# jwfoley/UniPeak

Measured on AMD Instinct MI355X. Metric: genome Gbp/s for KDE smoothing + region scan on hg19, at 1/2/4/8 MI355X, higher is better.
Workload: dtype f64

## Files before the change

include/unipeak_hip.h:

```cpp
#ifndef UNIPEAK_HIP_H
#define UNIPEAK_HIP_H

#include <stddef.h>
#include <stdint.h>

#ifdef __cplusplus
extern "C" {
#endif

#define UP_OK 0
#define UP_E_ARG (-1)
#define UP_E_HIP (-2)
#define UP_E_NOMEM (-3)
#define UP_E_STATE (-4)
#define UP_E_UNSUPPORTED (-5)
#define UP_E_NODEV (-6)
#define UP_E_INTERNAL (-7)

typedef struct up_ctx up_ctx;

typedef struct {
    uint16_t bw;
    uint16_t n_samples;
    int32_t nondir;
// ... 63 lines not shown
#define UP_MAX_IN_FLIGHT 5
int up_run_async(up_ctx *ctx);
int up_run_wait(up_ctx *ctx, uint64_t *n_regions);
int up_set_timing(up_ctx *ctx, int level);
int up_get_regions(up_ctx *ctx, up_region *out, uint32_t *counts, size_t cap);
int up_regions_view(up_ctx *ctx, const up_region **regions, const uint32_t **counts,
                    uint64_t *n);

int up_set_record_target(up_ctx *ctx, void *buf, uint64_t cap);
int up_host_register(up_ctx *ctx, void *ptr, uint64_t bytes);

int up_shift_scan(up_ctx *ctx, const uint64_t *region_idx, size_t n,
                  uint16_t max_shift, double *out);
int up_shift_best(up_ctx *ctx, const uint64_t *region_idx, size_t n,
                  uint16_t max_shift, uint16_t *best_shift, double *best_corr);

#define UP_INDEX_AUTO 0
#define UP_INDEX_NEVER 1
#define UP_INDEX_ALWAYS 2
int up_set_index_policy(up_ctx *ctx, int policy);
int up_invalidate_index(up_ctx *ctx);
int up_index_state(up_ctx *ctx, int *on, uint64_t *builds);
int up_last_stats_kind(up_ctx *ctx);
int up_scan_density(up_ctx *ctx, uint32_t *bytes_per_1024);
int up_hbm_copy_gbps(up_ctx *ctx, uint64_t bytes, int reps, double *gbps);
int up_timings(up_ctx *ctx, double *ms, int n);
int up_unit_profile(up_ctx *ctx, uint32_t unit, double *out_f, double *out_r,
                    uint32_t len);
#define UP_FLUSH_EVENT 0xFFFFFFFFu
int up_set_profile_capture(up_ctx *ctx, int on);
int up_unit_replay_profile(up_ctx *ctx, uint32_t unit, uint32_t *resync, uint64_t *n,
                           uint32_t *event, uint32_t *pos, double *score, uint64_t cap);
int up_unit_profile_range(up_ctx *ctx, uint32_t unit, uint64_t first, uint32_t count,
                          double *out_f, double *out_r);

#define UP_TIR_HOST 0xFFFFFFFFu
typedef struct up_tir up_tir;
int up_tir_open(int hip_device, up_tir **out);
void up_tir_close(up_tir *h);
int up_tir_set_stream(up_tir *h, uint32_t stream, uint64_t n, const uint64_t *key,
                      const uint32_t *count, const uint8_t *forward);
int up_tir_query(up_tir *h, uint32_t n_streams, uint64_t n_regions, const uint32_t *contig,
                 const uint32_t *left, const uint32_t *right, const uint8_t *forward,
                 uint32_t *first, uint32_t *end, uint32_t *hits);
int up_tir_timings(up_tir *h, double *ms, int n);

// ... 14 lines not shown
```

unipeak_amd/capi.py:

```python
import ctypes
import os

import numpy as np

_HERE = os.path.dirname(os.path.abspath(__file__))
LIB_PATH = os.environ.get("UNIPEAK_LIB") or os.path.join(_HERE, "lib", "libunipeak_hip.so")

UP_OK = 0
MAX_IN_FLIGHT = 5


class UpError(RuntimeError):
    def __init__(self, code, msg):
        super().__init__(f"{msg} (code {code})")
        self.code = code


class Params(ctypes.Structure):
    _fields_ = [
        ("bw", ctypes.c_uint16),
        ("n_samples", ctypes.c_uint16),
        ("nondir", ctypes.c_int32),
        ("background", ctypes.c_double),
        ("region_thr", ctypes.c_double),
# ... 19 lines not shown
        ("close_pos", ctypes.c_uint32),
        ("peak_score", ctypes.c_double),
        ("kurtosis", ctypes.c_double),
        ("corr", ctypes.c_double),
    ]


REGION_DTYPE = np.dtype([
    ("unit", "<u4"), ("left", "<u4"), ("right", "<u4"), ("peak", "<u4"),
    ("sum", "<u4"), ("nonctl_sum", "<u4"), ("accepted", "<i4"), ("close_pos", "<u4"),
    ("peak_score", "<f8"), ("kurtosis", "<f8"), ("corr", "<f8")])
assert REGION_DTYPE.itemsize == ctypes.sizeof(Region)

_lib = None

EXPORTS = [
    "up_version", "up_track_bits", "up_strerror", "up_device_count", "up_kernel_weights", "up_open",
    "up_close", "up_set_params", "up_add_unit", "up_unit_count", "up_unit_pack",
    "up_unit_scatter", "up_unit_synth", "up_unit_synth_offset", "up_unit_synth_ex", "up_unit_tag_total", "up_unit_set_last_add", "up_unit_last_add",
    "up_reset_units", "up_run", "up_get_regions", "up_regions_view", "up_shift_scan", "up_shift_best",
    "up_timings", "up_scan_density", "up_unit_profile", "up_hbm_copy_gbps", "up_set_record_target",
    "up_host_register", "up_unit_profile_range", "up_run_async", "up_run_wait", "up_set_timing",
    "up_set_profile_capture", "up_unit_replay_profile",
    "up_set_index_policy", "up_invalidate_index", "up_index_state", "up_last_stats_kind",
    "up_tir_open", "up_tir_close", "up_tir_set_stream", "up_tir_query", "up_tir_timings",
    "up_cm_open", "up_cm_close", "up_cm_add", "up_cm_collect", "up_cm_timings",
]
TIR_HOST = 0xFFFFFFFF
INDEX_AUTO, INDEX_NEVER, INDEX_ALWAYS = 0, 1, 2


def load_library(path=LIB_PATH):
    global _lib
    if _lib is not None:
        return _lib
    if not os.path.exists(path):
        raise OSError(f"{path} not built: run `python __graft_entry__.py` / tools/build.py")
    L = ctypes.CDLL(path)
    c = ctypes
    vp, u32p = c.c_void_p, c.POINTER(c.c_uint32)
    sig = {
        "up_version": (c.c_int, []),
        "up_track_bits": (c.c_int, []),
        "up_strerror": (c.c_char_p, [c.c_int]),
        "up_device_count": (c.c_int, [c.POINTER(c.c_int)]),
        "up_kernel_weights": (c.c_int, [c.c_uint16, c.c_double, vp]),
        "up_open": (c.c_int, [c.c_int, c.POINTER(vp)]),
# ... 9 lines not shown
                                           c.c_uint32, c.c_int32, c.c_int32, c.c_int32, c.c_int32]),
        "up_unit_synth_ex": (c.c_int, [vp, c.c_uint32, c.c_int32, c.c_uint16, c.c_uint64,
                                       c.c_uint32, c.c_int32, c.c_int32, c.c_int32, c.c_int32,
                                       c.c_uint64]),
        "up_unit_tag_total": (c.c_int, [vp, c.c_uint32, c.c_int32, c.c_uint16,
                                        c.POINTER(c.c_uint64)]),
        "up_unit_set_last_add": (c.c_int, [vp, c.c_uint32, c.c_uint32]),
        "up_unit_last_add": (c.c_int, [vp, c.c_uint32, u32p]),
        "up_reset_units": (c.c_int, [vp]),
        "up_run": (c.c_int, [vp, c.POINTER(c.c_uint64)]),
        "up_run_async": (c.c_int, [vp]),
        "up_run_wait": (c.c_int, [vp, c.POINTER(c.c_uint64)]),
        "up_set_timing": (c.c_int, [vp, c.c_int]),
        "up_get_regions": (c.c_int, [vp, vp, vp, c.c_size_t]),
        "up_regions_view": (c.c_int, [vp, c.POINTER(vp), c.POINTER(vp), c.POINTER(c.c_uint64)]),
        "up_shift_scan": (c.c_int, [vp, vp, c.c_size_t, c.c_uint16, vp]),
        "up_shift_best": (c.c_int, [vp, vp, c.c_size_t, c.c_uint16, vp, vp]),
        "up_timings": (c.c_int, [vp, vp, c.c_int]),
        "up_scan_density": (c.c_int, [vp, u32p]),
        "up_set_index_policy": (c.c_int, [vp, c.c_int]),
        "up_invalidate_index": (c.c_int, [vp]),
        "up_index_state": (c.c_int, [vp, c.POINTER(c.c_int), c.POINTER(c.c_uint64)]),
        "up_last_stats_kind": (c.c_int, [vp]),
        "up_unit_profile": (c.c_int, [vp, c.c_uint32, vp, vp, c.c_uint32]),
        "up_hbm_copy_gbps": (c.c_int, [vp, c.c_uint64, c.c_int, c.POINTER(c.c_double)]),
        "up_set_record_target": (c.c_int, [vp, vp, c.c_uint64]),
        "up_host_register": (c.c_int, [vp, vp, c.c_uint64]),
        "up_unit_profile_range": (c.c_int, [vp, c.c_uint32, c.c_uint64, c.c_uint32, vp, vp]),
        "up_set_profile_capture": (c.c_int, [vp, c.c_int]),
        "up_unit_replay_profile": (c.c_int, [vp, c.c_uint32, u32p, c.POINTER(c.c_uint64), vp, vp, vp,
                                             c.c_uint64]),
        "up_tir_open": (c.c_int, [c.c_int, c.POINTER(vp)]),
        "up_tir_close": (None, [vp]),
        "up_tir_set_stream": (c.c_int, [vp, c.c_uint32, c.c_uint64, vp, vp, vp]),
        "up_tir_query": (c.c_int, [vp, c.c_uint32, c.c_uint64, vp, vp, vp, vp, vp, vp, vp]),
        "up_tir_timings": (c.c_int, [vp, vp, c.c_int]),
        "up_cm_open": (c.c_int, [c.c_int, c.c_uint32, vp, c.POINTER(vp)]),
        "up_cm_close": (None, [vp]),
        "up_cm_add": (c.c_int, [vp, c.c_uint64, vp, vp, vp, vp]),
        "up_cm_collect": (c.c_int, [vp, c.c_int, c.POINTER(c.c_uint64), vp, vp, vp, vp, c.c_uint64]),
        "up_cm_timings": (c.c_int, [vp, vp, c.c_int]),
    }
    for name, (res, args) in sig.items():
        fn = getattr(L, name)
        fn.restype = res
        fn.argtypes = args
# ... 163 lines not shown

    def host_register(self, ptr, nbytes):
        _ck(self.L.up_host_register(self.ctx, ctypes.c_void_p(ptr), nbytes))

    def hbm_copy_gbps(self, nbytes=1 << 30, reps=5):
        v = ctypes.c_double()
        _ck(self.L.up_hbm_copy_gbps(self.ctx, nbytes, reps, ctypes.byref(v)))
        return v.value

    def set_index_policy(self, policy):
        _ck(self.L.up_set_index_policy(self.ctx, int(policy)))

    def invalidate_index(self):
        _ck(self.L.up_invalidate_index(self.ctx))

    def index_state(self):
        on, b = ctypes.c_int(0), ctypes.c_uint64(0)
        _ck(self.L.up_index_state(self.ctx, ctypes.byref(on), ctypes.byref(b)))
        return bool(on.value), int(b.value)

    def last_k3_kind(self):
        return int(self.L.up_last_stats_kind(self.ctx))

    def scan_density(self):
        v = ctypes.c_uint32()
        _ck(self.L.up_scan_density(self.ctx, ctypes.byref(v)))
        return v.value

    def timings(self):
        t = np.zeros(5, np.float64)
        _ck(self.L.up_timings(self.ctx, t.ctypes.data, 5))
        return t

    def profile(self, unit, length):
        f = np.zeros(length, np.float64)
        r = np.zeros(length, np.float64)
        _ck(self.L.up_unit_profile(self.ctx, unit, f.ctypes.data, r.ctypes.data, length))
        return f, r

    def profile_range(self, unit, first, count):
        f = np.zeros(count, np.float64)
        r = np.zeros(count, np.float64)
        _ck(self.L.up_unit_profile_range(self.ctx, unit, first, count, f.ctypes.data, r.ctypes.data))
        return f, r

    def profile_kernel_ms(self):
# ... 101 lines not shown
```

unipeak_amd/csrc/api.hip:

```cpp
#include <hip/hip_runtime.h>

#include <algorithm>
#include <unordered_map>
#include <chrono>
#include <cmath>
#include <condition_variable>
#include <deque>
#include <cstdio>
#include <cstring>
#include <map>
#include <mutex>
#include <thread>
#include <vector>

#include "../../include/unipeak_hip.h"
#include "kernels.h"

#include "kernels.hip"
#include "stats1.hip"
#include "emulate.hip"
#include "q11place.hip"
#include "wide.hip"

namespace upk {
const void *scan_kernel_nh1(int, bool, bool, int);
const void *scan_kernel_nh2(int, bool, bool, int);
const void *scan_kernel_nh3(int, bool, bool, int);
const void *scan_kernel_nh4(int, bool, bool, int);
const void *scan_kernel_nh5(int, bool, bool, int);
const void *scan_kernel_nh6(int, bool, bool, int);
const void *scan_kernel_nh7(int, bool, bool, int);
const void *scan_kernel_nh8(int, bool, bool, int);
const void *stats_kernel_nh1(int, bool, int);
const void *stats_kernel_nh2(int, bool, int);
const void *stats_kernel_nh3(int, bool, int);
const void *stats_kernel_nh4(int, bool, int);
const void *stats_kernel_nh5(int, bool, int);
const void *stats_kernel_nh6(int, bool, int);
const void *stats_kernel_nh7(int, bool, int);
const void *stats_kernel_nh8(int, bool, int);
const void *shift_kernel_nh1(int);
const void *shift_kernel_nh2(int);
const void *shift_kernel_nh3(int);
const void *shift_kernel_nh4(int);
const void *shift_kernel_nh5(int);
const void *shift_kernel_nh6(int);
const void *shift_kernel_nh7(int);
const void *shift_kernel_nh8(int);
static int window_nh(int bw) { return (bw + 64) / 64; }
static const void *scan_kernel_for(int bw, int pool, bool nd, bool prof, int mode) {
    switch (window_nh(bw)) {
    case 1: return scan_kernel_nh1(pool, nd, prof, mode);
    case 2: return scan_kernel_nh2(pool, nd, prof, mode);
    case 3: return scan_kernel_nh3(pool, nd, prof, mode);
    case 4: return scan_kernel_nh4(pool, nd, prof, mode);
    case 5: return scan_kernel_nh5(pool, nd, prof, mode);
    case 6: return scan_kernel_nh6(pool, nd, prof, mode);
    case 7: return scan_kernel_nh7(pool, nd, prof, mode);
    default: return scan_kernel_nh8(pool, nd, prof, mode);
    }
}
static const void *stats_kernel_for(int bw, int pool, bool nd, int one) {
    switch (window_nh(bw)) {
    case 1: return stats_kernel_nh1(pool, nd, one);
    case 2: return stats_kernel_nh2(pool, nd, one);
    case 3: return stats_kernel_nh3(pool, nd, one);
    case 4: return stats_kernel_nh4(pool, nd, one);
    case 5: return stats_kernel_nh5(pool, nd, one);
    case 6: return stats_kernel_nh6(pool, nd, one);
    case 7: return stats_kernel_nh7(pool, nd, one);
    default: return stats_kernel_nh8(pool, nd, one);
    }
// ... 76 lines not shown
        hipError_t e = hipHostMalloc((void **)&p, cap * sizeof(T), hipHostMallocMapped | hipHostMallocCoherent);
        if (e != hipSuccess) return e;
        e = hipHostGetDevicePointer((void **)&dev, p, 0);
        if (e == hipSuccess) n = cap;
        return e;
    }
    void release() {
        if (p) (void)hipHostFree(p);
        p = dev = nullptr;
        n = 0;
    }
};

constexpr int kSlots = UP_MAX_IN_FLIGHT;

}

struct up_ctx {
    int dev = 0;
    int ncu = 0;
    int k1a_per_cu = 3;
    int k1b_per_cu = 0;
    int k3_per_cu = 0;
    bool k3_one = true;
    bool use_graphs = true;
    hipStream_t k1a_stream = nullptr;
    hipStream_t chain[4] = {};
    int n_chain = 3;
    uint64_t nlaunch = 0;
    hipStream_t stream = nullptr;
    bool have_params = false;
    up_params p{};
    std::vector<uint8_t> ctl;
    std::vector<double> coef, kern;
    std::vector<int32_t> nc;
    DevBuf<double> d_kern, d_coef;
    DevBuf<int32_t> d_nc;
    DevBuf<uint8_t> d_ctl;
    DevBuf<uint32_t> d_wscreen;
    uint32_t wskip = 0;
    float fw[kScrHalo + 1] = {};
    float fthr = 0.f;
    bool q_ok = false;
    double q_alpha = 0.0, q_delta = 1.0;
    uint32_t qno = 0, qyes = 0;
    uint32_t ovf_max_all = 0;
// ... 39 lines not shown
        DevBuf<double> d_corr;
        void release() {
            d_info.release(); d_rec.release(); d_ovf_count.release(); d_ovf_rec.release(); d_head.release();
            d_cnt.release(); d_nreg.release(); d_bsum.release(); d_starts.release(); d_ends.release();
            d_runit.release(); d_peak_pos.release(); d_xlist.release(); d_xcount.release();
            d_xwcount.release(); d_xref.release(); d_peak_val.release(); d_spk.release(); d_corr.release();
        }
        uint8_t *target = nullptr;
        void *target_hostp = nullptr;
        uint64_t target_cap = 0;
        uint8_t *req_target = nullptr;
        void *req_target_hostp = nullptr;
        uint64_t req_target_cap = 0, req_last_nreg = 0;
        uint64_t req_reg_cap = 0;
        uint32_t req_ovf_cap = 0;
        int req_tl = 0;
        bool req_q11 = false;
        bool req_q11_place = false;
        bool lpending = false;
        int lrc = 0;
        uint64_t cap = 0;
        uint32_t ovf_cap = 0;
        int tl = 0;
        int k3_kind = -1;
        std::chrono::steady_clock::time_point t0;
        hipEvent_t ev[5] = {};
        hipEvent_t done = nullptr;
    } pass[kSlots];
    uint64_t seq_launched = 0, seq_done = 0;
    int cur_slot = 0;
    std::thread launcher;
    std::mutex lmu;
    std::condition_variable lcv;
    std::deque<int> lq;
    bool lbusy = false, lstop = false, use_launcher = true;
    hipEvent_t host_work = nullptr;
    DevBuf<uint32_t> d_resync, d_emu_n, d_emu_err, d_emu_counts, d_ring_hits, d_reg_hit, d_reg_hits;
    DevBuf<int32_t> d_unit_buffer;
    DevBuf<uint32_t> d_gunits, d_goff;
    DevBuf<uint32_t> d_gskip, d_gstop, d_emu_group;
    DevBuf<double> d_reg_f, d_reg_r;
    DevBuf<up_region> d_emu_out;
    DevBuf<double> d_ring_f, d_ring_r;
    bool prof_capture = false;
    uint64_t pf_cap = 1u << 20;
    DevBuf<uint32_t> d_pf_unit, d_pf_event, d_pf_pos;
// ... 29 lines not shown
    DevBuf<uint32_t> d_q11_stage_cnt;
    DevBuf<Q11Place> d_q11_tab;
    DevBuf<uint64_t> d_q11_scr;
    DevBuf<Q11Edit> d_q11_edit;
    DevBuf<uint32_t> d_q11_st, d_q11_en, d_q11_src;
    std::vector<std::pair<uint64_t, uint64_t>> q11_rep;
    std::vector<up_region> h_regions;
    std::vector<uint32_t> h_counts;
    std::vector<uint8_t> h_emulated;
    HostBuf<uint32_t> hp_head[kSlots];
    HostBuf<up_region> hp_regions[kSlots];
    HostBuf<uint32_t> hp_counts[kSlots];
    HostBuf<unsigned long long> hp_status[kSlots];
    void *target_hostp = nullptr;
    HostBuf<uint32_t> hp_scat[2];
    hipEvent_t scat_ev[2] = {};
    int scat_i = 0;
    uint64_t reg_cap = 1u << 16;
    uint8_t *target = nullptr;
    uint64_t target_cap = 0;
    void *target_host = nullptr;
    std::vector<void *> host_regs;
    uint64_t last_nreg = 0;
    int last_k3_kind = -1;
};

static bool busy(const up_ctx *c) { return c && c->seq_launched != c->seq_done; }

static void index_stale(up_ctx *c) { c->passes_on_tracks = 0; }

static void sync_all(up_ctx *c) {
    (void)hipStreamSynchronize(c->stream);
    (void)hipStreamSynchronize(c->k1a_stream);
    for (auto st : c->chain)
        if (st) (void)hipStreamSynchronize(st);
}

#define HIPCHK(x)                                                                   \
    do {                                                                            \
        hipError_t e_ = (x);                                                        \
        if (e_ != hipSuccess) {                                                     \
            fprintf(stderr, "unipeak_hip: %s failed: %s (%s:%d)\n", #x,             \
                    hipGetErrorString(e_), __FILE__, __LINE__);                     \
            return e_ == hipErrorOutOfMemory ? UP_E_NOMEM : UP_E_HIP;               \
        }                                                                           \
    } while (0)
// ... 20 lines not shown
int up_set_index_policy(up_ctx *c, int policy) {
    if (!c || policy < UP_INDEX_AUTO || policy > UP_INDEX_ALWAYS) return UP_E_ARG;
    if (busy(c)) return UP_E_STATE;
    c->index_policy = policy;
    return UP_OK;
}

int up_invalidate_index(up_ctx *c) {
    if (!c) return UP_E_ARG;
    if (busy(c)) return UP_E_STATE;
    for (Unit &u : c->units) u.cs_dirty = u.pool_dirty = true;
    index_stale(c);
    return UP_OK;
}

int up_index_state(up_ctx *c, int *on, uint64_t *builds) {
    if (!c) return UP_E_ARG;
    if (on) *on = c->index_on ? 1 : 0;
    if (builds) *builds = c->index_builds;
    return UP_OK;
}

int up_last_stats_kind(up_ctx *c) { return c ? c->last_k3_kind : -1; }

const char *up_strerror(int code) {
    switch (code) {
    case UP_OK: return "ok";
    case UP_E_ARG: return "bad argument";
    case UP_E_HIP: return "HIP runtime error";
    case UP_E_NOMEM: return "device memory exhausted";
    case UP_E_STATE: return "call out of order";
    case UP_E_UNSUPPORTED: return "configuration outside the GPU path";
    case UP_E_NODEV: return "no HIP device";
    case UP_E_INTERNAL: return "internal consistency check failed";
    default: return "unknown error";
    }
}

int up_device_count(int *n) {
    if (!n) return UP_E_ARG;
    int c = 0;
    if (hipGetDeviceCount(&c) != hipSuccess) c = 0;
    *n = c;
    return UP_OK;
}

// ... 5 lines not shown
        const double x2 = x * x;
        w[j] = 3 * (1 - x2) / 4;
        acc += w[j];
    }
    const double scale = sum / acc;
    for (int j = 0; j < 2 * (int)bw + 1; ++j) w[j] *= scale;
    return UP_OK;
}

int up_open(int hip_device, up_ctx **out) {
    if (!out) return UP_E_ARG;
    int n = 0;
    if (hipGetDeviceCount(&n) != hipSuccess || n == 0) return UP_E_NODEV;
    if (hip_device < 0 || hip_device >= n) return UP_E_ARG;
    up_ctx *c = new up_ctx();
    c->dev = hip_device;
    HIPCHK(hipSetDevice(hip_device));
    HIPCHK(hipDeviceGetAttribute(&c->ncu, hipDeviceAttributeMultiprocessorCount, hip_device));
    if (const char *e = getenv("UNIPEAK_K1A_PER_CU")) c->k1a_per_cu = atoi(e);
    if (const char *e = getenv("UNIPEAK_GRAPHS")) c->use_graphs = e[0] != '0';
    if (const char *e = getenv("UNIPEAK_K1B_PER_CU")) c->k1b_per_cu = atoi(e);
    if (const char *e = getenv("UNIPEAK_K3_PER_CU")) c->k3_per_cu = atoi(e);
    if (const char *e = getenv("UNIPEAK_K3_ONE")) c->k3_one = atoi(e) != 0;
    if (const char *e = getenv("UNIPEAK_CHAINS")) c->n_chain = std::min(4, std::max(1, atoi(e)));
    if (const char *e = getenv("UNIPEAK_LAUNCHER")) c->use_launcher = e[0] != '0';
    {
        int least = 0, greatest = 0;
        HIPCHK(hipDeviceGetStreamPriorityRange(&least, &greatest));
        const char *ep = getenv("UNIPEAK_CTX_PRIO");
        HIPCHK(hipStreamCreateWithPriority(&c->stream, hipStreamNonBlocking,
                                           (ep && ep[0] == '0') ? least : greatest));
        const char *e = getenv("UNIPEAK_K1A_PRIO");
        HIPCHK(hipStreamCreateWithPriority(&c->k1a_stream, hipStreamNonBlocking,
                                           (e && e[0] == '0') ? least : greatest));
        for (int i = 0; i < c->n_chain; ++i) HIPCHK(hipStreamCreateWithFlags(&c->chain[i], hipStreamNonBlocking));
    }
    for (auto &e : c->ev) HIPCHK(hipEventCreate(&e));
    for (auto &ps : c->pass) {
        for (auto &e : ps.ev) HIPCHK(hipEventCreate(&e));
        HIPCHK(hipEventCreateWithFlags(&ps.done, hipEventDisableTiming));
        HIPCHK(hipEventCreateWithFlags(&ps.k1a_end, hipEventDisableTiming));
    }
    HIPCHK(hipEventCreateWithFlags(&c->host_work, hipEventDisableTiming));
    for (auto &e : c->scat_ev) HIPCHK(hipEventCreateWithFlags(&e, hipEventDisableTiming));
    *out = c;
    return UP_OK;
// ... 804 lines not shown
    static std::map<std::pair<const void *, size_t>, int> per_cu;
    int n = 0;
    {
        std::lock_guard<std::mutex> g(mu);
        auto it = per_cu.find({kernel, lds});
        if (it != per_cu.end()) {
            n = it->second;
        } else {
            if (hipOccupancyMaxActiveBlocksPerMultiprocessor(&n, kernel, threads, lds) != hipSuccess || n < 1) n = 1;
            per_cu[{kernel, lds}] = n;
        }
    }
    return (uint32_t)n * (uint32_t)(c->ncu > 0 ? c->ncu : 256);
}

template <bool PROF, int MODE>
static void dispatch_scan(up_ctx *c, hipStream_t st, const ScanParams &P, uint32_t b, uint32_t e) {
    constexpr bool kScr = MODE == kModeScreen || MODE == kModeScreenF;
    const size_t lds = kScr ? kScreenLds : MODE == kModeExact ? kExactLds : kScanLds;
    const void *k = scan_kernel_for(P.bw, pool_mode(c), c->p.nondir != 0, PROF, MODE);
    uint32_t blocks = resident_blocks(c, k, lds);
    if (MODE == kModeExact) {
        if (c->k1b_per_cu > 0) blocks = (uint32_t)c->k1b_per_cu * (uint32_t)(c->ncu > 0 ? c->ncu : 256);
    } else {
        if (kScr) {
            const uint32_t cap = (uint32_t)c->k1a_per_cu * (uint32_t)(c->ncu > 0 ? c->ncu : 256);
            if (c->k1a_per_cu > 0 && cap < blocks) blocks = cap;
        }
        const uint32_t need = (e - b + 3) / 4;
        if (need < blocks) blocks = need;
        if (blocks > kMaxK1aWaves / 4) blocks = kMaxK1aWaves / 4;
        if (blocks == 0) return;
    }
    ScanParams Q = P;
    if (kScr) {
        c->k1a_waves = 4 * blocks;
        c->k1a_xcap = Q.xcap = (e - b + c->k1a_waves - 1) / c->k1a_waves;
    }
    void *args[] = {&Q, &b, &e};
    (void)hipLaunchKernel(k, dim3(blocks), dim3(256), args, lds, st);
}

static StatParams stat_params(up_ctx *c, up_ctx::Pass &ps) {
    StatParams P{};
    P.units = c->d_units.p;
    P.S = c->p.n_samples;
    P.nnc = (int32_t)c->nc.size();
    P.nc = c->d_nc.p;
    P.is_control = c->d_ctl.p;
    P.coef = c->d_coef.p;
    P.kern = c->d_kern.p;
    P.bw = c->p.bw;
    P.nondir = c->p.nondir;
    P.want_corr = c->p.want_corr || c->p.corr_thr > -1;
    P.region_thr = c->p.region_thr;
    P.kurt_thr = c->p.kurt_thr;
    P.corr_thr = c->p.corr_thr;
    P.hit_thr = c->p.hit_thr;
    P.starts = ps.d_starts.p;
    P.ends = ps.d_ends.p;
    P.reg_unit = ps.d_runit.p;
    P.peak_pos = nullptr;
// ... 501 lines not shown
    if (!scatter) return UP_OK;
    HIPCHK(c->d_q11_st.ensure(dcap + 1));
    HIPCHK(c->d_q11_en.ensure(dcap + 1));
    HIPCHK(c->d_q11_src.ensure(dcap + 1));
    const unsigned blocks = (unsigned)std::min<uint64_t>((ps.cap + 255) / 256 + 1, 4096);
    hipLaunchKernelGGL(q11_scatter_kernel, dim3(blocks), dim3(256), 0, st, c->d_q11_stage.p,
                       c->d_q11_stage_cnt.p, ps.d_nreg.p, (int)c->p.n_samples, c->d_q11_tab.p, out, oc, dcap,
                       c->d_q11_st.p, c->d_q11_en.p, c->d_q11_src.p);
    HIPCHK(hipGetLastError());
    return UP_OK;
}

static int enqueue_rest(up_ctx *c, int slot, const ScanParams &SP, const StatParams &P, uint64_t cap,
                        uint32_t k1a_waves, uint32_t k1a_xcap, bool events) {
    up_ctx::Pass &ps = c->pass[slot];
    const uint32_t ns = c->nstrips;
    const uint32_t nsb = (ns + kSegBlock - 1) / kSegBlock;
    if (!ps.req_q11 && c->p.bw <= kMaxBw) {
        if (k1a_waves) {
            hipLaunchKernelGGL(xref_kernel, dim3(1), dim3(1024), 0, ps.stream, ps.d_xwcount.p, k1a_waves,
                               k1a_xcap, ps.d_xref.p, ps.d_xcount.p);
            HIPCHK(hipGetLastError());
        }
        dispatch_scan<false, kModeExact>(c, ps.stream, SP, 0, ns);
        HIPCHK(hipGetLastError());
    }
    if (events) HIPCHK(hipEventRecord(ps.ev[2], ps.stream));
    unsigned long long *thdr = (unsigned long long *)ps.target;
    if (int r = launch_seg_count_head(c, slot)) return r;
    hipLaunchKernelGGL(seg_compact_kernel, dim3(nsb), dim3(kSegBlock), 0, ps.stream, c->d_units.p,
                       (uint32_t)c->units.size(), ps.d_info.p, ps.d_cnt.p, ps.d_bsum.p, ps.d_rec.p,
                       ps.d_ovf_rec.p, ps.ovf_cap, ps.d_starts.p, ps.d_ends.p, ps.d_runit.p, ps.d_peak_pos.p,
                       ps.d_peak_val.p, ns, (uint64_t)cap, ps.d_ovf_count.p, ps.d_xcount.p, ps.d_nreg.p,
                       c->hp_status[slot].dev, thdr);
    HIPCHK(hipGetLastError());
    if (events) HIPCHK(hipEventRecord(ps.ev[3], ps.stream));
    dispatch_stats(c, ps.stream, P, std::max<uint64_t>(ps.req_last_nreg, 1024));
    HIPCHK(hipGetLastError());
    if (ps.req_q11_place)
        if (int r = q11_place(c, slot, ps.stream, nullptr, true)) return r;
    if (events) HIPCHK(hipEventRecord(ps.ev[4], ps.stream));
    return UP_OK;
}

static int launch_pass(up_ctx *c, int slot) {
    const uint32_t ns = c->nstrips;
    const int S = c->p.n_samples;
// ... 87 lines not shown
        P.cap = cap;
        const unsigned blocks = (unsigned)std::min<uint64_t>((ns + 3) / 4, 4096);
        hipLaunchKernelGGL(proc_runs_kernel, dim3(std::max(1u, blocks)), dim3(256), 0, s1, SP);
    } else {
        if (c->p.bw > kMaxBw) {
            graph = false;
            const unsigned blocks = std::max(1u, std::min<uint32_t>(ns, 8192));
            const int pm = pool_mode(c);
            if (pm == 0) hipLaunchKernelGGL(wide_kernel<0>, dim3(blocks), dim3(64), 0, s1, SP);
            else if (pm == 1) hipLaunchKernelGGL(wide_kernel<1>, dim3(blocks), dim3(64), 0, s1, SP);
            else hipLaunchKernelGGL(wide_kernel<2>, dim3(blocks), dim3(64), 0, s1, SP);
        } else {
            if (plane_scan(c) || window_nh(c->p.bw) > 4) dispatch_scan<false, kModeScreen>(c, s1, SP, 0, ns);
            else dispatch_scan<false, kModeScreenF>(c, s1, SP, 0, ns);
        }
    }
    HIPCHK(hipGetLastError());
    hipEvent_t k1a_end = ps.k1a_end;
    if (tl >= 1) k1a_end = ps.ev[1];
    HIPCHK(hipEventRecord(k1a_end, s1));
    HIPCHK(hipStreamWaitEvent(ps.stream, k1a_end, 0));
    const uint32_t kw = c->k1a_waves, kx = c->k1a_xcap;
    ps.k3_kind = k3_kind_for(c, P, std::max<uint64_t>(ps.req_last_nreg, 1024));
    if (!graph || tl >= 2) {
        if (int r = enqueue_rest(c, slot, SP, P, cap, kw, kx, tl >= 2)) return r;
        HIPCHK(hipEventRecord(ps.done, ps.stream));
        return UP_OK;
    }
    std::vector<uint8_t> key;
    key_add(key, SP);
    key_add(key, P);
    key_add(key, kw);
    key_add(key, kx);
    key_add(key, std::max<uint64_t>(ps.req_last_nreg, 1024));
    key_add(key, (uint32_t)c->units.size());
    key_add(key, ovf_cap);
    key_add(key, pool_mode(c));
    key_add(key, c->p.nondir);
    key_add(key, c->nc.size());
    key_add(key, c->hp_head[slot].dev);
    key_add(key, c->hp_status[slot].dev);
    key_add(key, ps.d_head.p);
    key_add(key, c->d_coef.p);
    key_add(key, ps.target);
    key_add(key, ps.d_cnt.p);
    key_add(key, ps.d_bsum.p);
    size_t gi = 0;
    while (gi < ps.graphs.size() && ps.graphs[gi].first != key) ++gi;
    if (gi == ps.graphs.size()) {
        HIPCHK(hipStreamBeginCapture(ps.stream, hipStreamCaptureModeThreadLocal));
        const int r = enqueue_rest(c, slot, SP, P, cap, kw, kx, false);
        hipGraph_t g = nullptr;
        const hipError_t e = hipStreamEndCapture(ps.stream, &g);
        if (r) {
            if (g) (void)hipGraphDestroy(g);
            return r;
// ... 94 lines not shown
        c->lcv.notify_one();
    } else if ((r = launch_pass(c, slot))) {
        sync_all(c);
        c->seq_done = c->seq_launched;
        return r;
    }
    ++c->seq_launched;
    ++c->passes_on_tracks;
    return UP_OK;
}

int up_run_wait(up_ctx *c, uint64_t *n_regions) {
    if (!c) return UP_E_ARG;
    if (!busy(c)) return UP_E_STATE;
    HIPCHK(hipSetDevice(c->dev));
    const int slot = (int)(c->seq_done % kSlots);
    up_ctx::Pass &ps = c->pass[slot];
    c->ran = false;
    c->nreg = 0;
    c->host_regions = false;
    c->q11_placed = false;
    c->cur_slot = slot;
    c->last_k3_kind = -1;
    if (c->units.empty()) {
        ++c->seq_done;
        if (n_regions) *n_regions = 0;
        c->ran = true;
        return UP_OK;
    }
    auto fail = [&](int rc) {
        launcher_drain(c);
        sync_all(c);
        c->seq_done = c->seq_launched;
        return rc;
    };
    {
        std::unique_lock<std::mutex> lk(c->lmu);
        c->lcv.wait(lk, [&] { return !ps.lpending; });
    }
    if (ps.lrc) return fail(ps.lrc);
    if (hipEventSynchronize(ps.done) != hipSuccess) return fail(UP_E_HIP);
    uint64_t nreg = 0;
    for (int attempt = 0;; ++attempt) {
        if (attempt == 3) return fail(UP_E_INTERNAL);
        const unsigned long long *st = c->hp_status[slot].p;
        if (st[2]) return fail(UP_E_INTERNAL);
// ... 11 lines not shown
                            "cycles load %llu scatter %llu; words with a flag %llu, flagged positions %llu, "
                            "words reaching thr/2 %llu\n",
                    c->nstrips, h[0], h[1], h[2], h[3], h[4], h[5], h[6], h[7]);
            fprintf(stderr, "unipeak_hip: K1b clocks: item %llu load %llu scatter %llu flags %llu items %llu "
                            "max wave %llu waves %llu (Q part of scatter %llu)\n", h[16], h[17], h[18], h[19],
                    h[20], h[21], h[22], h[23]);
            fprintf(stderr, "unipeak_hip: K1b items by exact blocks:");
            for (int k = 1; k <= 16; ++k) fprintf(stderr, " %d:%llu", k, h[8 + k]);
            fprintf(stderr, "\n");
        }
#endif
        if (!again) break;
        launcher_drain(c);
        if (hipDeviceSynchronize() != hipSuccess) return fail(UP_E_HIP);
        ps.req_reg_cap = c->reg_cap;
        ps.req_ovf_cap = c->ovf_cap;
        int r = launch_pass(c, slot);
        if (r) return fail(r);
        if (hipEventSynchronize(ps.done) != hipSuccess) return fail(UP_E_HIP);
    }
    c->nreg = nreg;
    c->last_nreg = nreg;
    c->last_k3_kind = ps.k3_kind;
    int r = ps.req_q11 ? UP_OK : replay_head_hits(c, slot);
    if (r) return fail(r);
    const int tl = ps.tl;
    float a = 0, b = 0, d = 0, x = 0;
    if (tl >= 1) (void)hipEventElapsedTime(&a, ps.ev[0], ps.ev[1]);
    if (tl >= 2) {
        (void)hipEventElapsedTime(&x, ps.ev[1], ps.ev[2]);
        (void)hipEventElapsedTime(&b, ps.ev[2], ps.ev[3]);
        (void)hipEventElapsedTime(&d, ps.ev[3], ps.ev[4]);
    }
    c->times[0] = (double)a + x;
    c->times[4] = x;
    c->times[1] = b;
    c->times[2] = d;
    c->times[3] = std::chrono::duration<double, std::milli>(std::chrono::steady_clock::now() - ps.t0).count();
    ++c->seq_done;
    c->ran = true;
    if (n_regions) *n_regions = c->nreg;
    return UP_OK;
}

static int replay_segments(up_ctx *c, std::vector<up_region> &emu, std::vector<uint32_t> &ecnt,
                           std::vector<uint64_t> &soff, std::vector<uint32_t> &keep) {
// ... 58 lines not shown
            if (sk > G_.k0 || (sk == G_.k0 && (int64_t)q.gstop[2 * l + 1] > G_.s)) continue;
        }
        kept[g] = 1;
        last[G_.b] = (int64_t)g;
    }
    keep.clear();
    for (uint32_t i = 0; i < emu.size(); ++i)
        if (kept[q.rgroup[i]]) keep.push_back(i);
    std::stable_sort(keep.begin(), keep.end(), [&](uint32_t x, uint32_t y) {
        if (emu[x].unit != emu[y].unit) return emu[x].unit < emu[y].unit;
        return q.rgroup[x] < q.rgroup[y];
    });
    return UP_OK;
}

static int run_replay(up_ctx *c, uint64_t *n_regions) {
    const auto t0 = std::chrono::steady_clock::now();
    HIPCHK(hipSetDevice(c->dev));
    c->ran = false;
    c->nreg = 0;
    c->host_regions = false;
    c->q11_placed = false;
    c->last_k3_kind = -1;
    c->h_regions.clear();
    c->h_counts.clear();
    c->h_emulated.clear();
    c->h_score_off.clear();
    int r = sync_units(c);
    if (r) return r;
    const uint32_t nu = (uint32_t)c->units.size();
    c->h_resync.assign(nu, 0);
    c->h_pf_off.assign(nu + 1, 0);
    up_ctx::Pass ps;
    ps.target = c->target;
    ps.target_hostp = c->target_hostp;
    ps.target_cap = c->target_cap;
    if (nu) {
        up_ctx::Pass &p0 = c->pass[0];
        HIPCHK(p0.d_head.ensure(nu));
        HIPCHK(hipMemsetD32Async((hipDeviceptr_t)p0.d_head.p, 1, nu, c->stream));
        std::vector<up_region> emu;
        std::vector<uint32_t> ecnt, resync;
        std::vector<uint64_t> soff;
        std::vector<uint32_t> order;
        static const bool whole = [] {
            const char *e = getenv("UNIPEAK_REPLAY_WHOLE");
// ... 514 lines not shown
```

unipeak_amd/csrc/nh_tu.hip:

```cpp
#include "kernels.hip"
#include "stats1.hip"

#ifndef UPK_NH_TU
#error "compile with -DUPK_NH_TU=1..8"
#endif

#define UPK_CAT2(a, b) a##b
#define UPK_CAT(a, b) UPK_CAT2(a, b)

namespace upk {

constexpr int kNH = UPK_NH_TU;

template <int POOL, bool ND>
static const void *scan_ptr(bool prof, int mode) {
    if (prof) return (const void *)scan_kernel<kNH, POOL, ND, true, kModeFused>;
    if constexpr (kNH <= 4) {
        if (mode == kModeScreenF) {
            if constexpr (POOL == 0 && !ND) return (const void *)k1a_fields_kernel<kNH>;
            return (const void *)scan_kernel<kNH, POOL, ND, false, kModeScreenF>;
        }
    }
    return mode == kModeExact ? (const void *)scan_kernel<kNH, POOL, ND, false, kModeExact>
                              : (const void *)scan_kernel<kNH, POOL, ND, false, kModeScreen>;
}

const void *UPK_CAT(scan_kernel_nh, UPK_NH_TU)(int pool, bool nd, bool prof, int mode) {
    if (nd) {
        if (pool == 0) return scan_ptr<0, true>(prof, mode);
        if (pool == 1) return scan_ptr<1, true>(prof, mode);
        return scan_ptr<2, true>(prof, mode);
    }
    if (pool == 0) return scan_ptr<0, false>(prof, mode);
    if (pool == 1) return scan_ptr<1, false>(prof, mode);
    return scan_ptr<2, false>(prof, mode);
}

const void *UPK_CAT(stats_kernel_nh, UPK_NH_TU)(int pool, bool nd, int one) {
    if (one == 2) return (const void *)stats1L_kernel<kNH>;
    if (one) return (const void *)stats1_kernel<kNH>;
    if (nd) {
        if (pool == 0) return (const void *)stats_kernel<kNH, 0, true>;
        if (pool == 1) return (const void *)stats_kernel<kNH, 1, true>;
        return (const void *)stats_kernel<kNH, 2, true>;
    }
    if (pool == 0) return (const void *)stats_kernel<kNH, 0, false>;
    if (pool == 1) return (const void *)stats_kernel<kNH, 1, false>;
    return (const void *)stats_kernel<kNH, 2, false>;
}

const void *UPK_CAT(shift_kernel_nh, UPK_NH_TU)(int pool) {
    if (pool == 0) return (const void *)shift_kernel<kNH, 0>;
    if (pool == 1) return (const void *)shift_kernel<kNH, 1>;
    return (const void *)shift_kernel<kNH, 2>;
}

}
```

Measured before the change: 8071.

## Add specialized one-wave exact-pass kernel with software-pipelined strip loads

Adds a dedicated exact1 kernel for the K1b exact pass, used when tracks are 2-bit, pooling and nondir are off, and q-mode applies. Each wave walks its work list, prefetching the next entries' headers and window data while computing the current one. It uses a prefix-sum quadratic key screen with a fallback to full kernel evaluation, and writes run records directly. The goal is to cut latency and generality overhead in the exact scan, at the cost of a second code path that must match the generic kernel's results.

```diff
diff --git a/include/unipeak_hip.h b/include/unipeak_hip.h
--- a/include/unipeak_hip.h
+++ b/include/unipeak_hip.h
@@ -109,6 +109,7 @@
 int up_invalidate_index(up_ctx *ctx);
 int up_index_state(up_ctx *ctx, int *on, uint64_t *builds);
 int up_last_stats_kind(up_ctx *ctx);
+int up_last_exact_kind(up_ctx *ctx);
 int up_scan_density(up_ctx *ctx, uint32_t *bytes_per_1024);
 int up_hbm_copy_gbps(up_ctx *ctx, uint64_t bytes, int reps, double *gbps);
 int up_timings(up_ctx *ctx, double *ms, int n);
diff --git a/unipeak_amd/capi.py b/unipeak_amd/capi.py
--- a/unipeak_amd/capi.py
+++ b/unipeak_amd/capi.py
@@ -65,7 +65,7 @@
     "up_timings", "up_scan_density", "up_unit_profile", "up_hbm_copy_gbps", "up_set_record_target",
     "up_host_register", "up_unit_profile_range", "up_run_async", "up_run_wait", "up_set_timing",
     "up_set_profile_capture", "up_unit_replay_profile",
-    "up_set_index_policy", "up_invalidate_index", "up_index_state", "up_last_stats_kind",
+    "up_set_index_policy", "up_invalidate_index", "up_index_state", "up_last_stats_kind", "up_last_exact_kind",
     "up_tir_open", "up_tir_close", "up_tir_set_stream", "up_tir_query", "up_tir_timings",
     "up_cm_open", "up_cm_close", "up_cm_add", "up_cm_collect", "up_cm_timings",
 ]
@@ -121,6 +121,7 @@
         "up_invalidate_index": (c.c_int, [vp]),
         "up_index_state": (c.c_int, [vp, c.POINTER(c.c_int), c.POINTER(c.c_uint64)]),
         "up_last_stats_kind": (c.c_int, [vp]),
+        "up_last_exact_kind": (c.c_int, [vp]),
         "up_unit_profile": (c.c_int, [vp, c.c_uint32, vp, vp, c.c_uint32]),
         "up_hbm_copy_gbps": (c.c_int, [vp, c.c_uint64, c.c_int, c.POINTER(c.c_double)]),
         "up_set_record_target": (c.c_int, [vp, vp, c.c_uint64]),
@@ -330,6 +331,9 @@
     def last_k3_kind(self):
         return int(self.L.up_last_stats_kind(self.ctx))
 
+    def last_exact_kind(self):
+        return int(self.L.up_last_exact_kind(self.ctx))
+
     def scan_density(self):
         v = ctypes.c_uint32()
         _ck(self.L.up_scan_density(self.ctx, ctypes.byref(v)))
diff --git a/unipeak_amd/csrc/api.hip b/unipeak_amd/csrc/api.hip
--- a/unipeak_amd/csrc/api.hip
+++ b/unipeak_amd/csrc/api.hip
@@ -18,6 +18,7 @@
 
 #include "kernels.hip"
 #include "stats1.hip"
+#include "exact1.hip"
 #include "emulate.hip"
 #include "q11place.hip"
 #include "wide.hip"
@@ -31,6 +32,14 @@
 const void *scan_kernel_nh6(int, bool, bool, int);
 const void *scan_kernel_nh7(int, bool, bool, int);
 const void *scan_kernel_nh8(int, bool, bool, int);
+const void *exact1_kernel_nh1();
+const void *exact1_kernel_nh2();
+const void *exact1_kernel_nh3();
+const void *exact1_kernel_nh4();
+const void *exact1_kernel_nh5();
+const void *exact1_kernel_nh6();
+const void *exact1_kernel_nh7();
+const void *exact1_kernel_nh8();
 const void *stats_kernel_nh1(int, bool, int);
 const void *stats_kernel_nh2(int, bool, int);
 const void *stats_kernel_nh3(int, bool, int);
@@ -48,6 +57,18 @@
 const void *shift_kernel_nh7(int);
 const void *shift_kernel_nh8(int);
 static int window_nh(int bw) { return (bw + 64) / 64; }
+static const void *exact1_kernel_for(int bw) {
+    switch (window_nh(bw)) {
+    case 1: return exact1_kernel_nh1();
+    case 2: return exact1_kernel_nh2();
+    case 3: return exact1_kernel_nh3();
+    case 4: return exact1_kernel_nh4();
+    case 5: return exact1_kernel_nh5();
+    case 6: return exact1_kernel_nh6();
+    case 7: return exact1_kernel_nh7();
+    default: return exact1_kernel_nh8();
+    }
+}
 static const void *scan_kernel_for(int bw, int pool, bool nd, bool prof, int mode) {
     switch (window_nh(bw)) {
     case 1: return scan_kernel_nh1(pool, nd, prof, mode);
@@ -170,6 +191,8 @@
     int k1a_per_cu = 3;
     int k1b_per_cu = 0;
     int k3_per_cu = 0;
+    int k1b_blocks = 0;
+    bool k1b_one = true;
     bool k3_one = true;
     bool use_graphs = true;
     hipStream_t k1a_stream = nullptr;
@@ -255,6 +278,7 @@
         uint64_t cap = 0;
         uint32_t ovf_cap = 0;
         int tl = 0;
+        int k1b_kind = -1;
         int k3_kind = -1;
         std::chrono::steady_clock::time_point t0;
         hipEvent_t ev[5] = {};
@@ -330,6 +354,7 @@
     void *target_host = nullptr;
     std::vector<void *> host_regs;
     uint64_t last_nreg = 0;
+    int last_k1b_kind = -1;
     int last_k3_kind = -1;
 };
 
@@ -396,6 +421,7 @@
 }
 
 int up_last_stats_kind(up_ctx *c) { return c ? c->last_k3_kind : -1; }
+int up_last_exact_kind(up_ctx *c) { return c ? c->last_k1b_kind : -1; }
 
 const char *up_strerror(int code) {
     switch (code) {
@@ -447,6 +473,8 @@
     if (const char *e = getenv("UNIPEAK_K1B_PER_CU")) c->k1b_per_cu = atoi(e);
     if (const char *e = getenv("UNIPEAK_K3_PER_CU")) c->k3_per_cu = atoi(e);
     if (const char *e = getenv("UNIPEAK_K3_ONE")) c->k3_one = atoi(e) != 0;
+    if (const char *e = getenv("UNIPEAK_K1B_ONE")) c->k1b_one = atoi(e) != 0;
+    if (const char *e = getenv("UNIPEAK_K1B_BLOCKS")) c->k1b_blocks = std::max(0, atoi(e));
     if (const char *e = getenv("UNIPEAK_CHAINS")) c->n_chain = std::min(4, std::max(1, atoi(e)));
     if (const char *e = getenv("UNIPEAK_LAUNCHER")) c->use_launcher = e[0] != '0';
     {
@@ -1297,6 +1325,7 @@
     uint32_t blocks = resident_blocks(c, k, lds);
     if (MODE == kModeExact) {
         if (c->k1b_per_cu > 0) blocks = (uint32_t)c->k1b_per_cu * (uint32_t)(c->ncu > 0 ? c->ncu : 256);
+        if (c->k1b_blocks > 0) blocks = (uint32_t)c->k1b_blocks;
     } else {
         if (kScr) {
             const uint32_t cap = (uint32_t)c->k1a_per_cu * (uint32_t)(c->ncu > 0 ? c->ncu : 256);
@@ -1313,6 +1342,25 @@
         c->k1a_xcap = Q.xcap = (e - b + c->k1a_waves - 1) / c->k1a_waves;
     }
     void *args[] = {&Q, &b, &e};
+    (void)hipLaunchKernel(k, dim3(blocks), dim3(256), args, lds, st);
+}
+
+static int k1b_kind_for(const up_ctx *c) {
+    return c->k1b_one && kTB == 2 && pool_mode(c) == 0 && c->p.nondir == 0 && c->p.bw <= kMaxBw && q_mode(c) ? 1 : 0;
+}
+
+static void dispatch_exact(up_ctx *c, hipStream_t st, const ScanParams &P, uint32_t ns) {
+    if (k1b_kind_for(c) == 0) {
+        dispatch_scan<false, kModeExact>(c, st, P, 0, ns);
+        return;
+    }
+    const void *k = exact1_kernel_for(P.bw);
+    const size_t lds = exact1_lds(P.bw, window_nh(P.bw));
+    uint32_t blocks = resident_blocks(c, k, lds);
+    if (c->k1b_per_cu > 0) blocks = (uint32_t)c->k1b_per_cu * (uint32_t)(c->ncu > 0 ? c->ncu : 256);
+    if (c->k1b_blocks > 0) blocks = (uint32_t)c->k1b_blocks;
+    ScanParams Q = P;
+    void *args[] = {&Q};
     (void)hipLaunchKernel(k, dim3(blocks), dim3(256), args, lds, st);
 }
 
@@ -1860,7 +1908,7 @@
                                k1a_xcap, ps.d_xref.p, ps.d_xcount.p);
             HIPCHK(hipGetLastError());
         }
-        dispatch_scan<false, kModeExact>(c, ps.stream, SP, 0, ns);
+        dispatch_exact(c, ps.stream, SP, ns);
         HIPCHK(hipGetLastError());
     }
     if (events) HIPCHK(hipEventRecord(ps.ev[2], ps.stream));
@@ -1994,6 +2042,8 @@
     HIPCHK(hipStreamWaitEvent(ps.stream, k1a_end, 0));
     const uint32_t kw = c->k1a_waves, kx = c->k1a_xcap;
     ps.k3_kind = k3_kind_for(c, P, std::max<uint64_t>(ps.req_last_nreg, 1024));
+    const int k1b_kind = (ps.req_q11 || c->p.bw > kMaxBw) ? -1 : k1b_kind_for(c);
+    ps.k1b_kind = k1b_kind;
     if (!graph || tl >= 2) {
         if (int r = enqueue_rest(c, slot, SP, P, cap, kw, kx, tl >= 2)) return r;
         HIPCHK(hipEventRecord(ps.done, ps.stream));
@@ -2004,6 +2054,9 @@
     key_add(key, P);
     key_add(key, kw);
     key_add(key, kx);
+    key_add(key, k1b_kind);
+    key_add(key, c->k1b_per_cu);
+    key_add(key, c->k1b_blocks);
     key_add(key, std::max<uint64_t>(ps.req_last_nreg, 1024));
     key_add(key, (uint32_t)c->units.size());
     key_add(key, ovf_cap);
@@ -2144,6 +2197,7 @@
     c->q11_placed = false;
     c->cur_slot = slot;
     c->last_k3_kind = -1;
+    c->last_k1b_kind = -1;
     if (c->units.empty()) {
         ++c->seq_done;
         if (n_regions) *n_regions = 0;
@@ -2201,6 +2255,7 @@
     c->nreg = nreg;
     c->last_nreg = nreg;
     c->last_k3_kind = ps.k3_kind;
+    c->last_k1b_kind = ps.k1b_kind;
     int r = ps.req_q11 ? UP_OK : replay_head_hits(c, slot);
     if (r) return fail(r);
     const int tl = ps.tl;
@@ -2305,6 +2360,7 @@
     c->host_regions = false;
     c->q11_placed = false;
     c->last_k3_kind = -1;
+    c->last_k1b_kind = -1;
     c->h_regions.clear();
     c->h_counts.clear();
     c->h_emulated.clear();
diff --git a/unipeak_amd/csrc/exact1.hip b/unipeak_amd/csrc/exact1.hip
--- /dev/null
+++ b/unipeak_amd/csrc/exact1.hip
@@ -0,0 +1,288 @@
+#pragma once
+
+namespace upk {
+
+__host__ __device__ constexpr int exact1_wave_words(int nh) { return kStepWords * kWave + 4 * (kStepWords + 2 * nh); }
+inline size_t exact1_lds(int bw, int nh) {
+    return (size_t)(2 * kKPad + 2 * bw + 2) * sizeof(double) + 4 * (size_t)exact1_wave_words(nh) * sizeof(uint32_t);
+}
+
+template <int NH>
+__global__ void __launch_bounds__(256) __attribute__((amdgpu_waves_per_eu(UPK_K1B_WPE))) exact1_kernel(ScanParams P) {
+    extern __shared__ double lds_[];
+    constexpr int SW = kStepWords;
+    constexpr int NWIN = SW + 2 * NH;
+    static_assert(kTB == 2 && NWIN <= 64, "2-bit tracks, one wave load per window");
+    const int bw = P.bw;
+    const int ktab_n = 2 * kKPad + 2 * bw + 2;
+    for (int i = threadIdx.x; i < ktab_n; i += blockDim.x) {
+        const int j = i - kKPad;
+        lds_[i] = (j >= 0 && j <= 2 * bw) ? P.kern[j] : 0.0;
+    }
+    __syncthreads();
+    const double *ktab = lds_ + kKPad;
+    uint32_t *keys = (uint32_t *)(lds_ + ktab_n) + (threadIdx.x >> 6) * exact1_wave_words(NH);
+    uint8_t *stage = (uint8_t *)(keys + SW * kWave);
+
+    const auto *units = cptr(P.units);
+    const int lane = threadIdx.x & 63;
+    const uint32_t wave = __builtin_amdgcn_readfirstlane(blockIdx.x * (blockDim.x >> 6) + (threadIdx.x >> 6));
+    const uint32_t nwaves = __builtin_amdgcn_readfirstlane(gridDim.x * (blockDim.x >> 6));
+    const int nc0 = cptr(P.nc)[0];
+    const uint32_t bw2 = (uint32_t)(bw * bw);
+    const int hadr = 4 * ((lane + bw) & 63), ladr = 4 * ((lane - bw - 1) & 63);
+    const bool hsel = ((((lane - bw) & 63) + bw - 64 * (NH - 1)) >> 6) != 0;
+    const bool lsel = ((((lane + bw + 1) & 63) - bw - 1 + 64 * NH) >> 6) != 0;
+    const uint32_t sh = fshift(lane);
+    const int wl = lane < NWIN ? lane : NWIN - 1;
+
+    const uint32_t n = __builtin_amdgcn_readfirstlane(P.xcount[0] + P.xcount[1]);
+    const auto *xref = cptr(P.xref);
+    uint32_t it = wave;
+    if (it >= n) return;
+
+    struct Hdr {
+        uint32_t strip, eb, cur;
+    };
+    struct Loc {
+        gu8 *tb;
+        uint32_t local, unstrips;
+    };
+    auto load_hdr = [&](uint32_t ei, Hdr &h, uint32_t &mch) {
+        const uint32_t *e = P.xlist + (uint64_t)ei * kXEntry;
+        const auto *es = cptr(e);
+        h.strip = es[0];
+        const uint32_t e1 = es[1];
+        h.eb = e1 & 0xFFFFu;
+        mch = (e[2 + (lane >> 1)] >> (16 * (lane & 1))) & 0xFFFFu;
+        h.cur = e1 >> 16;
+        if (h.cur == 0xFFFFu) h.cur = find_unit(units, P.nunits, h.strip);
+    };
+    auto load_loc = [&](const Hdr &h, Loc &l) {
+        const uint64_t base = units[h.cur].base, stride = units[h.cur].stride;
+        const uint32_t s0 = units[h.cur].strip0;
+        l.local = h.strip - s0;
+        l.unstrips = units[h.cur].nstrips;
+        l.tb = (gu8 *)base + (uint64_t)nc0 * stride + fbyte(kPadPos) + (uint64_t)l.local * kStripBytes;
+    };
+    auto win_load = [&](const Loc &l, int j) -> u32x4 {
+        return *((gu32x4 *)(l.tb + (int64_t)kWordBytes * (j * SW - NH)) + wl);
+    };
+    auto first_block = [](uint32_t eb) { return eb ? __builtin_ctz(eb) : 0; };
+
+    Hdr h0{}, h1{}, h2{};
+    Loc l0{}, l1{};
+    uint32_t m0 = 0, m1 = 0, m2 = 0, xr2 = 0;
+    load_hdr(xref[it], h0, m0);
+    load_loc(h0, l0);
+    if (it + nwaves < n) load_hdr(xref[it + nwaves], h1, m1);
+    if (it + 2 * nwaves < n) xr2 = xref[it + 2 * nwaves];
+    u32x4 wv = win_load(l0, first_block(h0.eb));
+
+    for (;;) {
+        const bool v1 = it + nwaves < n, v2 = it + 2 * nwaves < n;
+        if (v1) load_loc(h1, l1);
+        if (v2) load_hdr(xr2, h2, m2);
+        uint32_t xr3 = 0;
+        if (it + 3 * nwaves < n) xr3 = xref[it + 3 * nwaves];
+
+        const uint32_t strip = h0.strip;
+        const int64_t p0 = 1 + (int64_t)l0.local * kStrip;
+        RecList R_{0, 0, kInline};
+        uint64_t F0 = 0;
+        bool open = false;
+        int last = -2;
+        bool pk_ok = false;
+        uint32_t best = 0, bpos = 0;
+        bool btie = false;
+        auto run_key = [&]() { return btie ? (double)best + 0.5 : (double)best; };
+        auto close_run = [&](uint32_t end_pos) {
+            const double m = run_key();
+            rec_end(R_, end_pos, pk_ok ? bpos : 0u, m, P, strip, lane);
+            if (!pk_ok && lane == 0) {
+                P.spk[4ull * strip] = (uint64_t)__double_as_longlong(m);
+                P.spk[4ull * strip + 1] = bpos;
+            }
+            open = false;
+        };
+
+        for (uint32_t eb = h0.eb; eb;) {
+            const int j = __builtin_ctz(eb);
+            eb &= eb - 1u;
+            uint32_t lw = 0;
+#pragma unroll
+            for (int q = 0; q < 4; ++q) {
+                const uint64_t bq = __ballot(((m0 >> (4 * q)) & 0xFu) != 0u) >> (4 * j);
+#pragma unroll
+                for (int i = 0; i < 4; ++i) lw |= (uint32_t)((bq >> i) & 1ull) << (4 * i + q);
+            }
+            const int64_t x0 = p0 + 64 * (j * SW - NH);
+
+            const u32x4 v = wv;
+            __builtin_amdgcn_wave_barrier();
+            uint32_t ebits = 0;
+            if (lane < NWIN) {
+                *(u32x4 *)(stage + 16 * lane) = v;
+                ebits = fbig32(v.x) | fbig32(v.y) | fbig32(v.z) | fbig32(v.w);
+            }
+            if (eb) wv = win_load(l0, __builtin_ctz(eb));
+            else if (v1) wv = win_load(l1, first_block(h1.eb));
+            __builtin_amdgcn_fence(__ATOMIC_RELEASE, "wavefront");
+            __builtin_amdgcn_wave_barrier();
+            __builtin_amdgcn_fence(__ATOMIC_ACQUIRE, "wavefront");
+            uint32_t wf[NWIN];
+#pragma unroll
+            for (int w = 0; w < NWIN; ++w) wf[w] = ((uint32_t)stage[kWordBytes * w + fbyte(lane)] >> sh) & kTMask;
+            if (__ballot(ebits != 0u)) {
+                const UnitDesc U = units[h0.cur];
+                resolve_escapes<NWIN>(wf, U, (uint32_t)nc0, x0, lane);
+            }
+
+            uint32_t anykey = 0;
+            uint32_t ln = (uint32_t)lane;
+            asm volatile("" : "+v"(ln));
+            typedef const volatile __attribute__((address_space(3))) double lds_vd;
+            lds_vd *vk = (lds_vd *)ktab;
+            {
+                uint32_t P0[NWIN], P1[NWIN], P2[NWIN];
+                uint32_t c0 = 0, c1 = 0, c2 = 0;
+                uint32_t nd = lw;
+#pragma unroll
+                for (int d = 1; d <= 2 * NH; ++d) nd |= lw << d;
+                WordLoop<0, NWIN>::run([&](auto wc) {
+                    constexpr int w = decltype(wc)::value;
+                    uint64_t any = 0;
+                    if ((nd >> w) & 1u) {
+                        any = __ballot(nz(wf[w]));
+                    } else {
+                        c0 = c1 = c2 = 0u;
+                    }
+                    if (any == 0) {
+                        P0[w] = c0;
+                        P1[w] = c1;
+                        P2[w] = c2;
+                    } else {
+                        const uint32_t c = wf[w];
+                        const uint32_t jj = 64u * w + ln;
+                        const uint32_t s0 = wave_scan_u32(c), s1 = wave_scan_u32(c * jj),
+                                       s2 = wave_scan_u32(c * (jj * jj));
+                        P0[w] = s0 + c0;
+                        P1[w] = s1 + c1;
+                        P2[w] = s2 + c2;
+                        c0 += rl_u(s0, 63);
+                        c1 += rl_u(s1, 63);
+                        c2 += rl_u(s2, 63);
+                    }
+                    constexpr int k = w - 2 * NH;
+                    if constexpr (k >= 0) {
+                        if ((lw >> k) & 1u) {
+                            auto win = [&](const uint32_t (&Pa)[NWIN]) {
+                                const uint32_t hi = (uint32_t)__builtin_amdgcn_ds_bpermute(
+                                    hadr, (int)(hsel ? Pa[k + 2 * NH] : Pa[k + 2 * NH - 1]));
+                                const uint32_t lo = (uint32_t)__builtin_amdgcn_ds_bpermute(
+                                    ladr, (int)(lsel ? Pa[k + 1] : Pa[k]));
+                                return hi - lo;
+                            };
+                            const uint32_t W0 = win(P0), W1 = win(P1), W2 = win(P2);
+                            const uint32_t i = 64u * (k + NH) + ln;
+                            const uint32_t q = bw2 * W0 - (i * i) * W0 + 2u * i * W1 - W2;
+                            double f = 0.0;
+                            if (__ballot(q > P.qno && q < P.qyes)) {
+                                WordLoop<0, 2 * NH + 1>::run([&](auto dc) {
+                                    constexpr int d = decltype(dc)::value - NH;
+                                    uint64_t m = __ballot(nz(wf[k + NH + d])) & win_mask(d, bw);
+                                    while (m) {
+                                        int hb[kHB];
+                                        double hc[kHB], kv[kHB];
+                                        next_hits(m, wf[k + NH + d], hb, hc);
+#pragma unroll
+                                        for (int h = 0; h < kHB; ++h)
+                                            kv[h] = vk[lane + (bw - 64 * d - hb[h])];
+#pragma unroll
+                                        for (int h = 0; h < kHB; ++h) f = f + kv[h] * hc[h];
+                                    }
+                                });
+                            }
+                            const bool fl = q >= P.qyes || (q > P.qno && f >= P.thr);
+                            const uint32_t key = fl ? q : 0u;
+                            keys[64 * k + lane] = key;
+                            anykey |= key;
+                        }
+                    }
+                });
+            }
+            if (__ballot(anykey != 0u) || open) {
+                __builtin_amdgcn_fence(__ATOMIC_RELEASE, "wavefront");
+                __builtin_amdgcn_wave_barrier();
+                __builtin_amdgcn_fence(__ATOMIC_ACQUIRE, "wavefront");
+#pragma unroll 1
+                for (uint32_t lm = lw; lm; lm &= lm - 1u) {
+                    const int k = __builtin_ctz(lm);
+                    const int g = j * SW + k;
+                    const int64_t wpos = p0 + 64 * g;
+                    if (open && g != last + 1) close_run((uint32_t)(p0 + 64 * (last + 1) - 1));
+                    last = g;
+                    const uint32_t sck = keys[64 * k + lane];
+                    const uint64_t F = __ballot(sck != 0u);
+                    if (g == 0) F0 = F;
+                    if (open && !(F & 1ull)) close_run((uint32_t)(wpos - 1));
+                    uint64_t st = F & ~((F << 1) | ((open || g == 0) ? 1ull : 0ull));
+                    while (st) {
+                        const int b = __builtin_ctzll(st);
+                        st &= st - 1;
+                        rec_start(R_, (uint32_t)(wpos + b), P, strip, lane);
+                    }
+                    uint64_t rem = F;
+                    while (rem) {
+                        const int a = __builtin_ctzll(rem);
+                        const uint64_t up = ~(rem >> a);
+                        const int len = up ? __builtin_ctzll(up) : 64 - a;
+                        rem = len + a >= 64 ? 0ull : rem & (~0ull << (a + len));
+                        const bool in = lane >= a && lane < a + len;
+                        const uint32_t kq = in ? sck : 0u;
+                        const uint32_t mq = wave_max_u32(kq);
+                        const uint64_t at = __ballot(kq == mq);
+                        if (!(a == 0 && open)) {
+                            best = mq;
+                            bpos = (uint32_t)(wpos + __builtin_ctzll(at));
+                            btie = (at & (at - 1)) != 0;
+                            pk_ok = g != 0 || a != 0;
+                        } else if (mq > best) {
+                            best = mq;
+                            bpos = (uint32_t)(wpos + __builtin_ctzll(at));
+                            btie = (at & (at - 1)) != 0;
+                        } else if (mq == best) {
+                            btie = true;
+                        }
+                        open = true;
+                        if (a + len < 64) close_run((uint32_t)(wpos + a + len - 1));
+                    }
+                }
+                __builtin_amdgcn_wave_barrier();
+            }
+        }
+        if (open && last != kStripWords - 1) close_run((uint32_t)(p0 + 64 * (last + 1) - 1));
+        if (open) {
+            if (lane == 0) {
+                P.spk[4ull * strip + 2] = (uint64_t)__double_as_longlong(run_key());
+                P.spk[4ull * strip + 3] = bpos;
+            }
+        }
+        const uint64_t info = (uint64_t)R_.ns | ((uint64_t)R_.ne << 16) | ((F0 & 1ull) << 32) |
+                              ((uint64_t)open << 33) | ((uint64_t)(l0.local == 0) << 34) |
+                              ((uint64_t)(l0.local + 1 == l0.unstrips) << 35) |
+                              ((uint64_t)(R_.slot != kInline) << 36);
+        if (lane == 0) P.strip_info[strip] = info;
+
+        if (!v1) break;
+        it += nwaves;
+        h0 = h1;
+        l0 = l1;
+        m0 = m1;
+        h1 = h2;
+        m1 = m2;
+        xr2 = xr3;
+    }
+}
+
+}
diff --git a/unipeak_amd/csrc/nh_tu.hip b/unipeak_amd/csrc/nh_tu.hip
--- a/unipeak_amd/csrc/nh_tu.hip
+++ b/unipeak_amd/csrc/nh_tu.hip
@@ -1,5 +1,6 @@
 #include "kernels.hip"
 #include "stats1.hip"
+#include "exact1.hip"
 
 #ifndef UPK_NH_TU
 #error "compile with -DUPK_NH_TU=1..8"
@@ -36,6 +37,8 @@
     return scan_ptr<2, false>(prof, mode);
 }
 
+const void *UPK_CAT(exact1_kernel_nh, UPK_NH_TU)() { return (const void *)exact1_kernel<kNH>; }
+
 const void *UPK_CAT(stats_kernel_nh, UPK_NH_TU)(int pool, bool nd, int one) {
     if (one == 2) return (const void *)stats1L_kernel<kNH>;
     if (one) return (const void *)stats1_kernel<kNH>;
```

Result: faster. 8688 (median of 6 runs) (+7.6%).
